# RagnarGrootKoerkamp/astar-pairwise-aligner

Measured on AMD Instinct MI355X. Metric: DP cell-updates/sec (GCUPS), full bit-parallel DP, 100kbp@5% div, higher is better.
Workload: dtype u32

## Files before the change

### astar-pairwise-aligner_amd/csrc/slice_kernel.hpp

```cpp
#pragma once
#include <hip/hip_runtime.h>
#include <stdint.h>

#include "slice_job_order.hpp"

namespace pa {
namespace slice {

#ifndef PA_SLICE_CLOCK_TURNS
#define PA_SLICE_CLOCK_TURNS 15
#endif
#ifndef PA_SLICE_YIELD
#define PA_SLICE_YIELD 2
#endif
constexpr int kPad = 64;
constexpr int kErrSpin = 7;
constexpr uint32_t kSpinLimit = 1u << 22;

struct SliceGroup {
    uint64_t a_off;
    uint64_t b_off;
    uint64_t h_off;
    uint32_t h_stride;
    int32_t n;
    int32_t nstrips;
    int32_t npairs;
    uint32_t first_pos;
    uint32_t ev_first, ev_count;
    uint32_t pad_;
};
struct SliceEvent {
    int32_t col;
    uint32_t mask;
};
struct SlicePair {
    uint64_t a_off, b_off;
    int32_t n, m;
    uint32_t pair;
    uint32_t pad_;
};

typedef uint32_t pa_slice_u32x2 __attribute__((ext_vector_type(2)));
__device__ __forceinline__ uint32_t dpp_wave_shr1(uint32_t old_, uint32_t src) {
    return (uint32_t)__builtin_amdgcn_update_dpp((int)old_, (int)src, 0x138, 0xf, 0xf, false);
}
__device__ __forceinline__ uint32_t dpp_wave_rol1(uint32_t x) {
    return (uint32_t)__builtin_amdgcn_update_dpp((int)x, (int)x, 0x134, 0xf, 0xf, false);
}
__device__ __forceinline__ uint2 ld_boundary(const uint2* p) {
    const unsigned long long v = __hip_atomic_load((const unsigned long long*)p, __ATOMIC_RELAXED, __HIP_MEMORY_SCOPE_AGENT);
    return make_uint2((uint32_t)v, (uint32_t)(v >> 32));
}
__device__ __forceinline__ void st_boundary(uint2* p, uint32_t hp, uint32_t hm) {
    __hip_atomic_store((unsigned long long*)p, (unsigned long long)hp | ((unsigned long long)hm << 32), __ATOMIC_RELAXED, __HIP_MEMORY_SCOPE_AGENT);
}

#define PA_SLICE_ROW_PAIR(vpA, vmA, vpB, vmB, nb0A, nb1A, nb0B, nb1B, a0, a1, hpp, hmp, hpo, hmo)                                      \
    do {                                                                                                                                \
        uint32_t zA_, zB_, hmA_, hpA_;                                                                                                  \
        asm volatile(                                                                                                                   \
            "v_xor_b32 %[zA], %[a1_], %[nb1A_]\n\t"                                                                                     \
            "v_xor_b32 %[zB], %[a1_], %[nb1B_]\n\t"                                                                                     \
            "v_bitop3_b32 %[zA], %[a0_], %[nb0A_], %[zA] bitop3:0x28\n\t"                                                               \
            "v_bitop3_b32 %[zB], %[a0_], %[nb0B_], %[zB] bitop3:0x28\n\t"                                                               \
            "v_bitop3_b32 %[zA], %[zA], %[vmA_], %[hmp_] bitop3:0xfe\n\t"                                                               \
            "v_and_b32 %[hmA], %[zA], %[vpA_]\n\t"                                                                                      \
            "v_bitop3_b32 %[hpA], %[vmA_], %[zA], %[vpA_] bitop3:0xf1\n\t"                                                              \
            "v_bitop3_b32 %[zB], %[zB], %[vmB_], %[hmA] bitop3:0xfe\n\t"                                                                \
            "v_bitop3_b32 %[vpA_], %[hmp_], %[zA], %[hpp_] bitop3:0xf1\n\t"                                                             \
            "v_and_b32 %[hmB], %[zB], %[vpB_]\n\t"                                                                                      \
            "v_and_b32 %[vmA_], %[hpp_], %[zA]\n\t"                                                                                     \
            "v_bitop3_b32 %[hpB], %[vmB_], %[zB], %[vpB_] bitop3:0xf1\n\t"                                                              \
            "v_bitop3_b32 %[vpB_], %[hmA], %[zB], %[hpA] bitop3:0xf1\n\t"                                                               \
            "v_and_b32 %[vmB_], %[hpA], %[zB]"                                                                                          \
            : [zA] "=&v"(zA_), [zB] "=&v"(zB_), [hmA] "=&v"(hmA_), [hpA] "=&v"(hpA_), [hmB] "=&v"(hmo), [hpB] "=&v"(hpo),              \
              [vpA_] "+v"(vpA), [vmA_] "+v"(vmA), [vpB_] "+v"(vpB), [vmB_] "+v"(vmB)                                                    \
            : [a0_] "v"(a0), [a1_] "v"(a1), [nb0A_] "v"(nb0A), [nb1A_] "v"(nb1A), [nb0B_] "v"(nb0B), [nb1B_] "v"(nb1B), [hpp_] "v"(hpp), \
              [hmp_] "v"(hmp));                                                                                                         \
    } while (0)

#define PA_SLICE_ROW_ONE(vpA, vmA, nb0A, nb1A, a0, a1, hpp, hmp, hpo, hmo)                                                              \
    do {                                                                                                                                \
        uint32_t zA_;                                                                                                                   \
        asm volatile(                                                                                                                   \
            "v_xor_b32 %[zA], %[a1_], %[nb1A_]\n\t"                                                                                     \
            "v_bitop3_b32 %[zA], %[a0_], %[nb0A_], %[zA] bitop3:0x28\n\t"                                                               \
            "v_bitop3_b32 %[zA], %[zA], %[vmA_], %[hmp_] bitop3:0xfe\n\t"                                                               \
            "v_and_b32 %[hmA], %[zA], %[vpA_]\n\t"                                                                                      \
            "v_bitop3_b32 %[hpA], %[vmA_], %[zA], %[vpA_] bitop3:0xf1\n\t"                                                              \
            "v_bitop3_b32 %[vpA_], %[hmp_], %[zA], %[hpp_] bitop3:0xf1\n\t"                                                             \
            "v_and_b32 %[vmA_], %[hpp_], %[zA]"                                                                                          \
            : [zA] "=&v"(zA_), [hmA] "=&v"(hmo), [hpA] "=&v"(hpo), [vpA_] "+v"(vpA), [vmA_] "+v"(vmA)                                   \
            : [a0_] "v"(a0), [a1_] "v"(a1), [nb0A_] "v"(nb0A), [nb1A_] "v"(nb1A), [hpp_] "v"(hpp), [hmp_] "v"(hmp));                    \
    } while (0)

constexpr int kRingEntries = 256;
constexpr uint32_t kRingMask = (uint32_t)(kRingEntries - 1) * 16u;

#define PA_SLICE_FEED(hpp, hmp, ohp, ohm, hin, min_)                                                                                     \
    asm volatile(                                                                                                                       \
        "s_mov_b64 vcc, 1\n\t"                                                                                                          \
        "v_cndmask_b32_dpp %[hpp_], %[ohp_], %[hin_], vcc wave_shr:1 row_mask:0xf bank_mask:0xf bound_ctrl:0\n\t"                       \
        "v_cndmask_b32_dpp %[hmp_], %[ohm_], %[hmin_], vcc wave_shr:1 row_mask:0xf bank_mask:0xf bound_ctrl:0"                          \
        : [hpp_] "=&v"(hpp), [hmp_] "=&v"(hmp)                                                                                          \
        : [ohp_] "v"(ohp), [ohm_] "v"(ohm), [hin_] "v"(hin), [hmin_] "v"(min_)                                                          \
        : "vcc")

template <int R>
__global__ __launch_bounds__(64, 2) void slice_kernel(const SliceJob* __restrict__ jobs, int njobs, const SliceGroup* __restrict__ groups,
                                                      const SliceEvent* __restrict__ events, const uint2* __restrict__ A, const uint2* __restrict__ B,
                                                      uint2* H, uint2* V, uint32_t* ticket_err, unsigned long long* dbg) {
    __shared__ uint4 ring[kRingEntries];
    const int lane = (int)threadIdx.x;
    const uint32_t wave_slot = (uint32_t)__builtin_amdgcn_s_getreg((4 - 1) << 11 | 4) & 15u;
    for (;;) {
        uint32_t tk = 0;
        if (lane == 0) tk = atomicAdd(ticket_err, 1u);
        tk = (uint32_t)__builtin_amdgcn_readfirstlane((int)tk);
        if (tk >= (uint32_t)njobs) break;
        const SliceJob job = jobs[tk];
        const SliceGroup grp = groups[job.group];
        const unsigned long long t_job0 = dbg ? __builtin_amdgcn_s_memrealtime() : 0ull;
        unsigned long long t_parked = 0, n_parks = 0;
        [[maybe_unused]] bool waited_before = false;
        [[maybe_unused]] int slack = 0;
        const int s = (int)job.strip, n = grp.n;
        const bool has_in = s > 0, has_out = s + 1 < grp.nstrips;
        const uint2* Ag = A + grp.a_off + kPad;
        const size_t row0 = grp.b_off + ((size_t)s * 64 + (size_t)lane) * R;
        const uint2* Hin = H + grp.h_off + (size_t)(has_in ? s - 1 : 0) * grp.h_stride + kPad;
        uint2* Hout = H + grp.h_off + (size_t)(has_out ? s : 0) * grp.h_stride + kPad;
        const SliceEvent* ev = events + grp.ev_first;
        uint32_t nb0[R], nb1[R], vp[R], vm[R];
#pragma unroll
        for (int i = 0; i < R; ++i) {
            const uint2 b = B[row0 + i];
            nb0[i] = b.x;
            nb1[i] = b.y;
            vp[i] = ~0u;
            vm[i] = 0u;
        }
        constexpr int kWaitStep = 8;
        uint32_t a0 = 0, a1 = 0, o_hp = 0, o_hm = ~0u;
        uint32_t off = (lane == 63 && has_out) ? (uint32_t)(-lane) * 8u : 0x7FFFFFF0u;
        int cnt = 1 - lane;
        int cnt16 = cnt * 16;
        constexpr int kNoEvent = INT32_MIN;
        uint32_t ev_i = 0;
        int ev_col16 = ev[0].col * 16;
        const int nchunks = (n + 63 + 63) / 64;
        const __amdgpu_buffer_rsrc_t hrs = __builtin_amdgcn_make_buffer_rsrc((void*)Hout, 0, (int)((uint32_t)n * 8u), 0x00020000);
        unsigned long long nA = 0, nH = ~0ull;
        uint2 kA = Ag[lane], kH = make_uint2(~0u, 0u);
        if (has_in) kH = ld_boundary(Hin + lane);
        ring[kRingEntries - 64 + lane] = make_uint4(0u, 0u, 0u, ~0u);
        __builtin_amdgcn_s_waitcnt(0);
        for (int q = 0; q < nchunks; ++q) {
#if PA_SLICE_CLOCK_TURNS
            if ((((uint32_t)__builtin_amdgcn_s_memrealtime() >> PA_SLICE_CLOCK_TURNS) ^ wave_slot) & 1u) __builtin_amdgcn_s_setprio(1);
            else __builtin_amdgcn_s_setprio(0);
#else
            if (((uint32_t)q ^ wave_slot) & 1u) __builtin_amdgcn_s_setprio(1);
            else __builtin_amdgcn_s_setprio(0);
#endif
            uint2 cA = kA, cH = kH;
            const int col = q * 64 + lane;
            if (has_in) {
                uint32_t spins = 0;
                const unsigned long long t_p0 = dbg ? __builtin_amdgcn_s_memrealtime() : 0ull;
                while (col < n && (cH.x & cH.y) != 0u) {
                    __builtin_amdgcn_s_sleep(32);
                    cH = ld_boundary(Hin + col);
                    if (++spins > kSpinLimit) {
                        atomicCAS(ticket_err + 1, 0u, (uint32_t)kErrSpin);
                        cH = make_uint2(~0u, 0u);
                    }
                }
                const bool waited = __builtin_amdgcn_readfirstlane((int)(__ballot(spins != 0u) != 0ull)) != 0;
#if PA_SLICE_YIELD == 1
                if (waited) __builtin_amdgcn_s_setprio(0);
#elif PA_SLICE_YIELD == 2
                if (waited || waited_before) __builtin_amdgcn_s_setprio(0);
                waited_before = waited;
#elif PA_SLICE_YIELD >= 3
                slack = waited ? PA_SLICE_YIELD : (slack > 0 ? slack - 1 : 0);
                if (slack > 0) __builtin_amdgcn_s_setprio(0);
#endif
                if (dbg && waited) {
                    t_parked += __builtin_amdgcn_s_memrealtime() - t_p0;
                    n_parks += 1;
                }
                if (col < n) st_boundary(const_cast<uint2*>(Hin) + col, ~0u, ~0u);
            }
            ring[col & (kRingEntries - 1)] = make_uint4(cA.x, cA.y, cH.x, cH.y);
            uint4 r = *(const uint4*)((const char*)ring + ((uint32_t)(cnt16 - 16) & kRingMask));
            const int pcol = min(col + 64, n + kPad - 1);
            const bool more = q + 1 < nchunks;
            if (more) {
                asm volatile("global_load_dwordx2 %0, %1, off ; pa_prefetch_load" : "=v"(nA) : "v"(Ag + pcol) : "memory");
                if (has_in) asm volatile("global_load_dwordx2 %0, %1, off sc1 ; pa_prefetch_load" : "=v"(nH) : "v"(Hin + pcol) : "memory");
            }
            const int jend = min(64, n + 63 - q * 64);
            const int wait_at = more ? kWaitStep : -1;
            for (int j = 0; j < jend; ++j) {
                asm volatile("" : "+s"(j));
                if (j == wait_at) {
                    asm volatile("s_waitcnt vmcnt(8) ; pa_prefetch_wait" : "+v"(nA), "+v"(nH)::"memory");
                    kA = make_uint2((uint32_t)nA, (uint32_t)(nA >> 32));
                    if (has_in) kH = make_uint2((uint32_t)nH, (uint32_t)(nH >> 32));
                }
                uint32_t hpp, hmp;
                a0 = r.x;
                a1 = r.y;
                PA_SLICE_FEED(hpp, hmp, o_hp, o_hm, r.z, r.w);
#pragma unroll
                for (int i = 0; i + 1 < R; i += 2) {
                    uint32_t hpo, hmo;
                    PA_SLICE_ROW_PAIR(vp[i], vm[i], vp[i + 1], vm[i + 1], nb0[i], nb1[i], nb0[i + 1], nb1[i + 1], a0, a1, hpp, hmp, hpo, hmo);
                    hpp = hpo;
                    hmp = hmo;
                }
                if constexpr (R & 1) {
                    uint32_t hpo, hmo;
                    PA_SLICE_ROW_ONE(vp[R - 1], vm[R - 1], nb0[R - 1], nb1[R - 1], a0, a1, hpp, hmp, hpo, hmo);
                    hpp = hpo;
                    hmp = hmo;
                }
                o_hp = hpp;
                o_hm = hmp;
                r = *(const uint4*)((const char*)ring + ((uint32_t)cnt16 & kRingMask));
                {
                    const pa_slice_u32x2 d = {hpp, hmp};
                    __builtin_amdgcn_raw_buffer_store_b64(d, hrs, off, 0, 16);
                }
                off += 8u;
                if (cnt16 == ev_col16) {
                    const uint32_t mask = ev[ev_i].mask;
#pragma unroll
                    for (int i = 0; i < R; ++i) {
                        atomicOr(&V[row0 + i].x, vp[i] & mask);
                        atomicOr(&V[row0 + i].y, vm[i] & mask);
                        asm volatile("" ::: "memory");
                    }
                    ++ev_i;
                    ev_col16 = ev_i < grp.ev_count ? ev[ev_i].col * 16 : kNoEvent;
                    __builtin_amdgcn_s_waitcnt(0);
                }
                cnt16 += 16;
            }
        }
        if (dbg && lane == 0) {
            const unsigned long long dt = __builtin_amdgcn_s_memrealtime() - t_job0;
            atomicMin(dbg + 0, dt);
            atomicMax(dbg + 1, dt);
            atomicAdd(dbg + 2, dt);
            atomicAdd(dbg + 3, 1ull);
            atomicAdd(dbg + 4, t_parked);
            atomicAdd(dbg + 5, n_parks);
            if (s == 0) {
                atomicMin(dbg + 6, dt);
                atomicMax(dbg + 7, dt);
            }
            const uint32_t xcc = (uint32_t)__builtin_amdgcn_s_getreg((4 - 1) << 11 | 20) & 7u;
            atomicAdd(dbg + 8 + 2 * xcc, dt - t_parked);
            atomicAdd(dbg + 9 + 2 * xcc, 1ull);
        }
    }
}


__device__ __forceinline__ uint32_t slice_rank16(const uint4 v, int count, bool& invalid) {
    const uint32_t q[4] = {v.x, v.y, v.z, v.w};
    uint32_t w = 0;
#pragma unroll
    for (int k = 0; k < 16; ++k) {
        const int r = rank_acgt((uint8_t)(q[k >> 2] >> (8 * (k & 3))));
        if (k < count) {
            invalid |= r < 0;
            w |= (uint32_t)(r & 3) << (2 * k);
        }
    }
    return w;
}

__global__ __launch_bounds__(256) void slice_pack_a_kernel(const SliceGroup* __restrict__ groups, const SlicePair* __restrict__ spairs,
                                                           const uint8_t* __restrict__ a_cat, uint2* __restrict__ A, uint32_t* __restrict__ bad) {
    const SliceGroup grp = groups[blockIdx.y];
    const int lane = (int)(threadIdx.x & 63), q = (int)(blockIdx.x * 4 + (threadIdx.x >> 6));
    if ((long long)q * 32 >= (long long)grp.n) return;
    const int p = lane & 31, half = lane >> 5, c0 = 32 * q + 16 * half;
    uint32_t w = 0;
    bool invalid = false;
    if (p < grp.npairs) {
        const SlicePair sp = spairs[grp.first_pos + p];
        if (c0 < sp.n) w = slice_rank16(*(const uint4*)(a_cat + sp.a_off + c0), sp.n - c0, invalid);
    }
    if (invalid) atomicOr(bad, 1u);
    uint32_t a0 = 0, a1 = 0;
#pragma unroll
    for (int k = 0; k < 16; ++k) {
        const unsigned long long b0 = __ballot((w >> (2 * k)) & 1u), b1 = __ballot((w >> (2 * k + 1)) & 1u);
        if ((lane & 15) == k) {
            a0 = (lane & 16) ? (uint32_t)(b0 >> 32) : (uint32_t)b0;
            a1 = (lane & 16) ? (uint32_t)(b1 >> 32) : (uint32_t)b1;
        }
    }
    const int c = q * 32 + lane;
    if (lane < 32 && c < grp.n) A[grp.a_off + kPad + c] = make_uint2(a0, a1);
}

__global__ __launch_bounds__(256) void slice_pack_b_kernel(const SliceGroup* __restrict__ groups, const SlicePair* __restrict__ spairs,
                                                           const uint8_t* __restrict__ b_cat, uint2* __restrict__ B, int rows_per_strip,
                                                           uint32_t* __restrict__ bad) {
    const SliceGroup grp = groups[blockIdx.y];
    const int lane = (int)(threadIdx.x & 63), j = (int)(blockIdx.x * 4 + (threadIdx.x >> 6));
    if ((long long)j * 64 >= (long long)grp.nstrips * rows_per_strip) return;
    const int p = lane & 31, half = lane >> 5;
    const long long r0 = (long long)j * 64 + 32 * half;
    uint32_t x0 = 0, x1 = 0;
    bool invalid = false;
    if (p < grp.npairs) {
        const SlicePair sp = spairs[grp.first_pos + p];
#pragma unroll
        for (int h = 0; h < 2; ++h) {
            const long long r = r0 + 16 * h;
            if (r < (long long)sp.m) {
                const int count = (int)min((long long)sp.m - r, 16ll);
                const uint32_t w = slice_rank16(*(const uint4*)(b_cat + sp.b_off + r), count, invalid);
                const uint32_t real = count >= 16 ? ~0u : (1u << (2 * count)) - 1u, nw = ~w & real;
                uint32_t e = 0, o = 0;
#pragma unroll
                for (int k = 0; k < 16; ++k) {
                    e |= ((nw >> (2 * k)) & 1u) << k;
                    o |= ((nw >> (2 * k + 1)) & 1u) << k;
                }
                x0 |= e << (16 * h);
                x1 |= o << (16 * h);
            }
        }
    }
    if (invalid) atomicOr(bad, 1u);
    uint32_t nb0 = 0, nb1 = 0;
#pragma unroll
    for (int k = 0; k < 32; ++k) {
        const unsigned long long b0 = __ballot((x0 >> k) & 1u), b1 = __ballot((x1 >> k) & 1u);
        if ((lane & 31) == k) {
            nb0 = half ? (uint32_t)(b0 >> 32) : (uint32_t)b0;
            nb1 = half ? (uint32_t)(b1 >> 32) : (uint32_t)b1;
        }
    }
    B[grp.b_off + (size_t)j * 64 + lane] = make_uint2(nb0, nb1);
}

constexpr int kScoreSpan = 4096;
__global__ __launch_bounds__(64) void slice_score_kernel(const SliceGroup* __restrict__ groups, const SlicePair* __restrict__ spairs,
                                                         const uint2* __restrict__ V, int32_t* __restrict__ cost_out) {
    const SliceGroup grp = groups[blockIdx.x];
    const int lane = (int)threadIdx.x;
    int my_m = 0, my_n = 0;
    uint32_t my_pair = 0;
    if (lane < grp.npairs) {
        const SlicePair sp = spairs[grp.first_pos + lane];
        my_m = sp.m;
        my_n = sp.n;
        my_pair = sp.pair;
    }
    int max_m = my_m;
#pragma unroll
    for (int o = 32; o > 0; o >>= 1) max_m = max(max_m, __shfl_xor(max_m, o));
    const int lo = (int)blockIdx.y * kScoreSpan, hi = min(max_m, lo + kScoreSpan);
    if (lo >= max_m) return;
    int acc = blockIdx.y == 0 ? my_n : 0;
    for (int r0 = lo; r0 < hi; r0 += 64) {
        const int r = r0 + lane;
        uint2 v = make_uint2(0u, 0u);
        if (r < hi) v = V[grp.b_off + r];
        for (int p = 0; p < grp.npairs; ++p) {
            const int mp = __shfl(my_m, p);
            const bool in = r < mp;
            const int pos = __popcll(__ballot(in && ((v.x >> p) & 1u))), neg = __popcll(__ballot(in && ((v.y >> p) & 1u)));
            if (lane == p) acc += pos - neg;
        }
    }
    if (lane < grp.npairs && acc != 0) atomicAdd(&cost_out[my_pair], acc);
}

}
}
```

### astar-pairwise-aligner_amd/csrc/slice_unit.hip

```cpp
#include "slice_plan.hpp"

#include <algorithm>
#include <cmath>
#include <cstdio>
#include <cstdlib>
#include <memory>
#include <numeric>
#include <vector>

#include "pa_hip_internal.hpp"
#include "slice_kernel.hpp"

namespace pa {
namespace slice {

struct Plan {
    int R = 52;
    size_t pairs = 0;
    std::vector<SliceGroup> groups;
    std::vector<SliceJob> jobs;
    size_t a_elems = 0, b_elems = 0, h_elems = 0;
    unsigned max_col_blocks = 0, max_row_blocks = 0;
    double valu = 0, computed = 0;
    int chain = 0;
    bool h_dirty = false;
    DeviceBuf d_groups, d_events, d_jobs, d_spairs, d_A, d_B, d_V, d_H;
};

static int strips_for(size_t m, int R) { return (int)((m + (size_t)64 * R - 1) / ((size_t)64 * R)); }

static constexpr double kNsPerRowStep = 16.2, kNsStepOverhead = 11.6, kChainPenalty = 0.0015;

static constexpr int kDefaultChain = 1;
static int chain_setting() {
    const char* e = getenv("PA_SLICE_CHAIN");
    return e && *e ? std::max(0, atoi(e)) : kDefaultChain;
}
static int chain_in_flight(int chain, size_t slots, size_t ngroups, int longest) {
    return chain == 0 ? longest : std::min(std::max(chain, auto_chain(ngroups, longest, slots)), longest);
}

int choose_rows_per_lane(const size_t* a_len, const size_t* b_len, size_t pairs, double simds, double* est_ns) {
    if (const char* e = getenv("PA_SLICE")) {
        if (atoi(e) == 0) return 0;
    }
    size_t live = 0;
    for (size_t i = 0; i < pairs; ++i) {
        live += a_len[i] > 0 && b_len[i] > 0;
        if (a_len[i] >= (size_t(1) << 27) - 64 || b_len[i] >= (size_t(1) << 27)) return 0;
    }
    const bool forced = getenv("PA_SLICE") && atoi(getenv("PA_SLICE")) > 0;
    if ((live + 31) / 32 > 65535) return 0;
    if (live < 64 && !forced) return 0;
    std::vector<uint32_t> order;
    for (size_t i = 0; i < pairs; ++i)
        if (a_len[i] > 0 && b_len[i] > 0) order.push_back((uint32_t)i);
    std::sort(order.begin(), order.end(), [&](uint32_t x, uint32_t y) { return a_len[x] != a_len[y] ? a_len[x] < a_len[y] : (b_len[x] != b_len[y] ? b_len[x] < b_len[y] : x < y); });
    int best_r = 0;
    double best = -1;
    const double slots = simds * 2.0;
    for (const int R : kRowsPerLane) {
        if (forced && atoi(getenv("PA_SLICE")) > 1 && atoi(getenv("PA_SLICE")) != R) continue;
        double work = 0, longest = 0, jobs = 0;
        const size_t ngroups = (order.size() + 31) / 32;
        size_t m_max = 0;
        for (const uint32_t i : order) m_max = std::max(m_max, b_len[i]);
        const int S_max = strips_for(m_max, R);
        const int C = chain_in_flight(chain_setting(), (size_t)slots, ngroups, S_max);
        for (size_t g = 0; g * 32 < order.size(); ++g) {
            size_t n = 0, m = 0;
            for (size_t t = g * 32; t < std::min(order.size(), g * 32 + 32); ++t) {
                n = std::max(n, a_len[order[t]]);
                m = std::max(m, b_len[order[t]]);
            }
            const int S = strips_for(m, R);
            const double per_strip = ((double)n + 63.0) * (R * kNsPerRowStep + kNsStepOverhead) * (1.0 + kChainPenalty * (std::min(S, C) - 1));
            work += per_strip * S;
            jobs += S;
            longest = std::max(longest, per_strip + 128.0 * (S - 1) * (R * kNsPerRowStep + kNsStepOverhead));
        }
        const double waves = std::min(jobs, slots);
        const double speed = waves <= simds ? 1.165 : 1.0 + 0.165 * (slots - waves) / simds;
        const double rounds = jobs > slots ? std::ceil(jobs / slots) * (work / jobs) : work / waves;
        const double t = std::max(longest / 1.165, rounds / speed);
        if (best < 0 || t < best) {
            best = t;
            best_r = R;
        }
    }
    if (est_ns) *est_ns = best;
    return best_r;
}

Plan* create(const size_t* a_len, const size_t* b_len, size_t pairs, const size_t* a_off, const size_t* b_off, int rows_per_lane) {
    auto p = std::make_unique<Plan>();
    p->R = rows_per_lane;
    p->pairs = pairs;
    const int R = rows_per_lane;
    std::vector<uint32_t> order;
    for (size_t i = 0; i < pairs; ++i)
        if (a_len[i] > 0 && b_len[i] > 0) order.push_back((uint32_t)i);
    std::sort(order.begin(), order.end(), [&](uint32_t x, uint32_t y) { return a_len[x] != a_len[y] ? a_len[x] < a_len[y] : (b_len[x] != b_len[y] ? b_len[x] < b_len[y] : x < y); });
    std::vector<SlicePair> spairs(order.size());
    std::vector<SliceEvent> events;
    size_t a_at = 0, b_at = 0, h_at = 0;
    size_t max_n = 0, max_rows = 0;
    const size_t ngroups = (order.size() + 31) / 32;
    for (size_t gi = 0; gi < ngroups; ++gi) {
        const size_t g = ngroups - 1 - gi;
        SliceGroup grp{};
        grp.first_pos = (uint32_t)(g * 32);
        grp.npairs = (int32_t)std::min<size_t>(32, order.size() - g * 32);
        size_t n = 0, m = 0;
        for (int t = 0; t < grp.npairs; ++t) {
            const uint32_t i = order[g * 32 + t];
            n = std::max(n, a_len[i]);
            m = std::max(m, b_len[i]);
            spairs[g * 32 + t] = SlicePair{(uint64_t)a_off[i], (uint64_t)b_off[i], (int32_t)a_len[i], (int32_t)b_len[i], i, 0u};
        }
        grp.n = (int32_t)n;
        grp.nstrips = strips_for(m, R);
        grp.a_off = a_at;
        grp.b_off = b_at;
        grp.h_off = h_at;
        grp.h_stride = (uint32_t)(n + 2 * kPad);
        a_at += n + 2 * kPad;
        b_at += (size_t)grp.nstrips * 64 * R;
        h_at += (size_t)(grp.nstrips - 1) * grp.h_stride;
        grp.ev_first = (uint32_t)events.size();
        for (int t = 0; t < grp.npairs; ++t) {
            const int32_t col = (int32_t)a_len[order[g * 32 + t]];
            if (events.size() > grp.ev_first && events.back().col == col) events.back().mask |= 1u << t;
            else events.push_back(SliceEvent{col, 1u << t});
        }
        grp.ev_count = (uint32_t)events.size() - grp.ev_first;
        max_n = std::max(max_n, n);
        max_rows = std::max(max_rows, (size_t)grp.nstrips * 64 * R);
        p->valu += (double)grp.nstrips * ((double)n + 63.0) * (7.0 * R + kStepOverheadInstr);
        p->computed += (double)grp.nstrips * 64.0 * R * (double)n * 32.0;
        p->groups.push_back(grp);
    }
    {
        std::vector<int> nstrips;
        for (const SliceGroup& g : p->groups) nstrips.push_back(g.nstrips);
        const size_t slots = (size_t)device_cus() * 8;
        p->chain = chain_setting();
        p->jobs = job_order(nstrips, slots, p->chain);
    }
    p->a_elems = a_at;
    p->b_elems = b_at;
    p->h_elems = h_at;
    p->max_col_blocks = (unsigned)((max_n + 127) / 128);
    p->max_row_blocks = (unsigned)((max_rows / 64 + 3) / 4);
    if (p->groups.empty()) return p.release();
    if (events.empty()) events.push_back(SliceEvent{0, 0});
    if (!p->d_groups.alloc(p->groups.size() * sizeof(SliceGroup)) || !p->d_events.alloc(events.size() * sizeof(SliceEvent)) ||
        !p->d_jobs.alloc(p->jobs.size() * sizeof(SliceJob)) || !p->d_spairs.alloc(spairs.size() * sizeof(SlicePair)) || !p->d_A.alloc(a_at * 8) ||
        !p->d_B.alloc(b_at * 8) || !p->d_V.alloc(b_at * 8) || !p->d_H.alloc(std::max<size_t>(h_at, 8) * 8))
        return nullptr;
    if (!hip_ok(hipMemcpy(p->d_groups.ptr, p->groups.data(), p->groups.size() * sizeof(SliceGroup), hipMemcpyHostToDevice), "H2D slice groups") ||
        !hip_ok(hipMemcpy(p->d_events.ptr, events.data(), events.size() * sizeof(SliceEvent), hipMemcpyHostToDevice), "H2D slice events") ||
        !hip_ok(hipMemcpy(p->d_jobs.ptr, p->jobs.data(), p->jobs.size() * sizeof(SliceJob), hipMemcpyHostToDevice), "H2D slice jobs") ||
        !hip_ok(hipMemcpy(p->d_spairs.ptr, spairs.data(), spairs.size() * sizeof(SlicePair), hipMemcpyHostToDevice), "H2D slice pairs") ||
        !hip_ok(hipMemset(p->d_A.ptr, 0, a_at * 8), "memset slice A") ||
        (h_at && !hip_ok(hipMemset(p->d_H.ptr, 0xFF, h_at * 8), "memset slice boundaries")))
        return nullptr;
    return p.release();
}

void destroy(Plan* p) { delete p; }

void mark_clean(Plan* p) { p->h_dirty = false; }

template <int R>
static hipError_t launch_slice(int grid, hipStream_t s, const Plan* p, uint32_t* d_ticket_err, unsigned long long* dbg) {
    hipLaunchKernelGGL((slice_kernel<R>), dim3((unsigned)grid), dim3(64), 0, s, p->d_jobs.as<SliceJob>(), (int)p->jobs.size(), p->d_groups.as<SliceGroup>(),
                       p->d_events.as<SliceEvent>(), p->d_A.as<uint2>(), p->d_B.as<uint2>(), p->d_H.as<uint2>(), p->d_V.as<uint2>(), d_ticket_err, dbg);
    return hipGetLastError();
}

int run(Plan* p, hipStream_t s, const uint8_t* d_a, const uint8_t* d_b, uint32_t* d_bad, int32_t* d_costs, uint32_t* d_ticket_err, hipEvent_t ev0,
        hipEvent_t ev1) {
    if (!hip_ok(hipMemsetAsync(d_ticket_err, 0, 8, s), "memset slice ticket")) return PA_E_HIP;
    if (p->groups.empty()) {
        if (ev0 && (!hip_ok(hipEventRecord(ev0, s), "event") || !hip_ok(hipEventRecord(ev1, s), "event"))) return PA_E_HIP;
        return 0;
    }
    const unsigned G = (unsigned)p->groups.size();
    hipLaunchKernelGGL(slice_pack_a_kernel, dim3(p->max_col_blocks, G), dim3(256), 0, s, p->d_groups.as<SliceGroup>(), p->d_spairs.as<SlicePair>(), d_a,
                       p->d_A.as<uint2>(), d_bad);
    hipLaunchKernelGGL(slice_pack_b_kernel, dim3(p->max_row_blocks, G), dim3(256), 0, s, p->d_groups.as<SliceGroup>(), p->d_spairs.as<SlicePair>(), d_b,
                       p->d_B.as<uint2>(), 64 * p->R, d_bad);
    if (!hip_ok(hipGetLastError(), "slice transposes")) return PA_E_HIP;
    if (!hip_ok(hipMemsetAsync(p->d_V.ptr, 0, p->b_elems * 8, s), "memset slice V")) return PA_E_HIP;
    if (p->h_elems && p->h_dirty && !hip_ok(hipMemsetAsync(p->d_H.ptr, 0xFF, p->h_elems * 8, s), "memset slice boundaries")) return PA_E_HIP;
    p->h_dirty = true;
    int grid = (int)std::min<size_t>(p->jobs.size(), (size_t)device_cus() * 8);
    const int grid_cap = getenv("PA_SLICE_GRID") ? atoi(getenv("PA_SLICE_GRID")) : 0;
    if (grid_cap > 0) grid = std::min(grid, grid_cap);
    static const bool jobtimes = getenv("PA_SLICE_JOBTIMES") != nullptr;
    unsigned long long* dbg = nullptr;
    if (jobtimes && hipMalloc((void**)&dbg, 192) == hipSuccess) {
        const unsigned long long init[24] = {~0ull, 0, 0, 0, 0, 0, ~0ull, 0};
        if (hipMemcpyAsync(dbg, init, 192, hipMemcpyHostToDevice, s) != hipSuccess || hipStreamSynchronize(s) != hipSuccess) dbg = nullptr;
    }
    if (ev0 && !hip_ok(hipEventRecord(ev0, s), "event")) return PA_E_HIP;
    hipError_t e = hipSuccess;
    switch (p->R) {
        case 52: e = launch_slice<52>(grid, s, p, d_ticket_err, dbg); break;
        case 51: e = launch_slice<51>(grid, s, p, d_ticket_err, dbg); break;
        case 50: e = launch_slice<50>(grid, s, p, d_ticket_err, dbg); break;
        case 49: e = launch_slice<49>(grid, s, p, d_ticket_err, dbg); break;
        case 48: e = launch_slice<48>(grid, s, p, d_ticket_err, dbg); break;
        case 47: e = launch_slice<47>(grid, s, p, d_ticket_err, dbg); break;
        case 46: e = launch_slice<46>(grid, s, p, d_ticket_err, dbg); break;
        case 45: e = launch_slice<45>(grid, s, p, d_ticket_err, dbg); break;
        case 44: e = launch_slice<44>(grid, s, p, d_ticket_err, dbg); break;
        case 42: e = launch_slice<42>(grid, s, p, d_ticket_err, dbg); break;
        case 40: e = launch_slice<40>(grid, s, p, d_ticket_err, dbg); break;
        case 36: e = launch_slice<36>(grid, s, p, d_ticket_err, dbg); break;
        case 32: e = launch_slice<32>(grid, s, p, d_ticket_err, dbg); break;
        case 28: e = launch_slice<28>(grid, s, p, d_ticket_err, dbg); break;
        default: set_error("slice: no kernel for %d rows per lane", p->R); return PA_E_INTERNAL;
    }
    if (!hip_ok(e, "slice_kernel")) return PA_E_HIP;
    if (ev1 && !hip_ok(hipEventRecord(ev1, s), "event")) return PA_E_HIP;
    if (dbg) {
        unsigned long long h[24] = {0};
        if (hipMemcpyAsync(h, dbg, 192, hipMemcpyDeviceToHost, s) == hipSuccess && hipStreamSynchronize(s) == hipSuccess && h[3]) {
            std::fprintf(stderr, "[slice jobs] awake us per job by XCD:");
            for (int x = 0; x < 8; ++x) std::fprintf(stderr, " %d: %.0f (%llu)", x, h[9 + 2 * x] ? h[8 + 2 * x] * 0.01 / (double)h[9 + 2 * x] : 0.0, h[9 + 2 * x]);
            std::fprintf(stderr, "\n");
            std::fprintf(stderr, "[slice jobs] R %d chain %d: %llu jobs, us per job: min %.1f mean %.1f max %.1f (first strips: min %.1f max %.1f); asleep behind the strip above: %.2f %% of the job time, %.1f waits per job\n",
                         p->R, p->chain, h[3], h[0] * 0.01, h[2] * 0.01 / (double)h[3], h[1] * 0.01, h[6] * 0.01, h[7] * 0.01, 100.0 * (double)h[4] / (double)h[2], (double)h[5] / (double)h[3]);
        }
        (void)hipFree(dbg);
    }
    hipLaunchKernelGGL(slice_score_kernel, dim3(G, (p->max_row_blocks * 256u + kScoreSpan - 1) / kScoreSpan), dim3(64), 0, s, p->d_groups.as<SliceGroup>(), p->d_spairs.as<SlicePair>(), p->d_V.as<uint2>(), d_costs);
    if (!hip_ok(hipGetLastError(), "slice_score_kernel")) return PA_E_HIP;
    return 0;
}

Info info(const Plan* p) {
    Info i{};
    i.rows_per_lane = p->R;
    i.groups = p->groups.size();
    i.jobs = p->jobs.size();
    i.chain = p->chain;
    i.valu_instructions = p->valu;
    i.computed_rows_cells = p->computed;
    i.device_bytes = (double)(p->a_elems + 2 * p->b_elems + p->h_elems) * 8.0;
    i.boundary_bytes = (double)p->h_elems * 8.0;
    return i;
}

}
}
```

Before: 274,100.

## Use SWAR base ranking and swizzle-based 32x32 bit transpose in pack and score kernels

```diff
diff --git a/astar-pairwise-aligner_amd/csrc/slice_kernel.hpp b/astar-pairwise-aligner_amd/csrc/slice_kernel.hpp
--- a/astar-pairwise-aligner_amd/csrc/slice_kernel.hpp
+++ b/astar-pairwise-aligner_amd/csrc/slice_kernel.hpp
@@ -268,99 +268,130 @@
     }
 }
 
-
-__device__ __forceinline__ uint32_t slice_rank16(const uint4 v, int count, bool& invalid) {
-    const uint32_t q[4] = {v.x, v.y, v.z, v.w};
-    uint32_t w = 0;
-#pragma unroll
-    for (int k = 0; k < 16; ++k) {
-        const int r = rank_acgt((uint8_t)(q[k >> 2] >> (8 * (k & 3))));
-        if (k < count) {
-            invalid |= r < 0;
-            w |= (uint32_t)(r & 3) << (2 * k);
-        }
-    }
-    return w;
+#define PA_SLICE_T32_STAGES(X) X(16, 0x0000FFFFu) X(8, 0x00FF00FFu) X(4, 0x0F0F0F0Fu) X(2, 0x33333333u) X(1, 0x55555555u)
+
+template <int D>
+__device__ __forceinline__ uint32_t slice_t32_stage(uint32_t x, uint32_t keep_clear, int lane) {
+    const uint32_t y = (uint32_t)__builtin_amdgcn_ds_swizzle((int)x, (D << 10) | 0x1f);
+    const bool set = (lane & D) != 0;
+    const uint32_t keep = set ? ~keep_clear : keep_clear;
+    const uint32_t moved = __builtin_amdgcn_alignbit(y, y, set ? (uint32_t)D : (uint32_t)(32 - D));
+    return (x & keep) | (moved & ~keep);
+}
+__device__ __forceinline__ uint32_t slice_transpose32(uint32_t x, int lane) {
+#define PA_SLICE_T32_STAGE_(D, KEEP) x = slice_t32_stage<D>(x, KEEP, lane);
+    PA_SLICE_T32_STAGES(PA_SLICE_T32_STAGE_)
+#undef PA_SLICE_T32_STAGE_
+    return x;
+}
+
+constexpr int kPackTile = 128;
+
+__device__ __forceinline__ uint32_t slice_rank4(uint32_t x) {
+    const uint32_t s1 = x >> 1, s2 = x >> 2;
+    const uint32_t t = s2 & ~s1 & 0x01010101u;
+    const uint32_t letter = ((((x & 0x06060606u) | 0x41414141u) ^ t) | (t << 4));
+    const uint32_t d = x ^ letter;
+    const uint32_t bad = ((((d & 0x7f7f7f7fu) + 0x7f7f7f7fu) | d) >> 7) & 0x01010101u;
+    const uint32_t c0 = ((s1 ^ s2) & 0x01010101u) | bad, c1 = (s2 & 0x01010101u) | bad;
+    return (((c0 | (c1 << 4)) * 0x01020408u) >> 24) | (((bad * 0x01020408u) >> 24) << 8);
+}
+
+struct SliceTileBits {
+    uint32_t c0[2], c1[2], bad[2], valid[2];
+};
+__device__ __forceinline__ SliceTileBits slice_read_tile(const uint8_t* __restrict__ seq, int len, int pos0) {
+    uint4 v[4];
+#pragma unroll
+    for (int i = 0; i < 4; ++i) {
+        const int pos = pos0 + 64 * (i >> 1) + 16 * (i & 1);
+        v[i] = make_uint4(0u, 0u, 0u, 0u);
+        if (pos < len) v[i] = *(const uint4*)(seq + pos);
+    }
+    SliceTileBits t;
+#pragma unroll
+    for (int j = 0; j < 2; ++j) {
+        uint32_t c0 = 0, c1 = 0, bad = 0;
+#pragma unroll
+        for (int h = 0; h < 2; ++h) {
+            const uint32_t q[4] = {v[2 * j + h].x, v[2 * j + h].y, v[2 * j + h].z, v[2 * j + h].w};
+#pragma unroll
+            for (int k = 0; k < 4; ++k) {
+                const uint32_t r = slice_rank4(q[k]);
+                c0 |= (r & 15u) << (16 * h + 4 * k);
+                c1 |= ((r >> 4) & 15u) << (16 * h + 4 * k);
+                bad |= (r >> 8) << (16 * h + 4 * k);
+            }
+        }
+        const int left = min(max(len - (pos0 + 64 * j), 0), 32);
+        t.c0[j] = c0;
+        t.c1[j] = c1;
+        t.bad[j] = bad;
+        t.valid[j] = left >= 32 ? ~0u : (1u << left) - 1u;
+    }
+    return t;
 }
 
 __global__ __launch_bounds__(256) void slice_pack_a_kernel(const SliceGroup* __restrict__ groups, const SlicePair* __restrict__ spairs,
                                                            const uint8_t* __restrict__ a_cat, uint2* __restrict__ A, uint32_t* __restrict__ bad) {
     const SliceGroup grp = groups[blockIdx.y];
-    const int lane = (int)(threadIdx.x & 63), q = (int)(blockIdx.x * 4 + (threadIdx.x >> 6));
-    if ((long long)q * 32 >= (long long)grp.n) return;
-    const int p = lane & 31, half = lane >> 5, c0 = 32 * q + 16 * half;
-    uint32_t w = 0;
-    bool invalid = false;
+    const int lane = (int)(threadIdx.x & 63);
+    const long long tile = (long long)blockIdx.x * 4 + (threadIdx.x >> 6);
+    if (tile * kPackTile >= (long long)grp.n) return;
+    const int c_tile = (int)tile * kPackTile, p = lane & 31, half = lane >> 5;
+    int len = 0;
+    const uint8_t* seq = a_cat;
     if (p < grp.npairs) {
         const SlicePair sp = spairs[grp.first_pos + p];
-        if (c0 < sp.n) w = slice_rank16(*(const uint4*)(a_cat + sp.a_off + c0), sp.n - c0, invalid);
-    }
-    if (invalid) atomicOr(bad, 1u);
-    uint32_t a0 = 0, a1 = 0;
-#pragma unroll
-    for (int k = 0; k < 16; ++k) {
-        const unsigned long long b0 = __ballot((w >> (2 * k)) & 1u), b1 = __ballot((w >> (2 * k + 1)) & 1u);
-        if ((lane & 15) == k) {
-            a0 = (lane & 16) ? (uint32_t)(b0 >> 32) : (uint32_t)b0;
-            a1 = (lane & 16) ? (uint32_t)(b1 >> 32) : (uint32_t)b1;
-        }
-    }
-    const int c = q * 32 + lane;
-    if (lane < 32 && c < grp.n) A[grp.a_off + kPad + c] = make_uint2(a0, a1);
+        len = sp.n;
+        seq = a_cat + sp.a_off;
+    }
+    const SliceTileBits t = slice_read_tile(seq, len, c_tile + 32 * half);
+    if (((t.bad[0] & t.valid[0]) | (t.bad[1] & t.valid[1])) != 0u) atomicOr(bad, 1u);
+#pragma unroll
+    for (int j = 0; j < 2; ++j) {
+        const uint32_t a0 = slice_transpose32(t.c0[j] & t.valid[j], lane), a1 = slice_transpose32(t.c1[j] & t.valid[j], lane);
+        const int c = c_tile + 64 * j + lane;
+        if (c < grp.n) A[grp.a_off + kPad + c] = make_uint2(a0, a1);
+    }
 }
 
 __global__ __launch_bounds__(256) void slice_pack_b_kernel(const SliceGroup* __restrict__ groups, const SlicePair* __restrict__ spairs,
                                                            const uint8_t* __restrict__ b_cat, uint2* __restrict__ B, int rows_per_strip,
                                                            uint32_t* __restrict__ bad) {
     const SliceGroup grp = groups[blockIdx.y];
-    const int lane = (int)(threadIdx.x & 63), j = (int)(blockIdx.x * 4 + (threadIdx.x >> 6));
-    if ((long long)j * 64 >= (long long)grp.nstrips * rows_per_strip) return;
-    const int p = lane & 31, half = lane >> 5;
-    const long long r0 = (long long)j * 64 + 32 * half;
-    uint32_t x0 = 0, x1 = 0;
-    bool invalid = false;
+    const int lane = (int)(threadIdx.x & 63);
+    const long long tile = (long long)blockIdx.x * 4 + (threadIdx.x >> 6);
+    const long long rows = (long long)grp.nstrips * rows_per_strip;
+    if (tile * kPackTile >= rows) return;
+    const int r_tile = (int)tile * kPackTile, p = lane & 31, half = lane >> 5;
+    int len = 0;
+    const uint8_t* seq = b_cat;
     if (p < grp.npairs) {
         const SlicePair sp = spairs[grp.first_pos + p];
-#pragma unroll
-        for (int h = 0; h < 2; ++h) {
-            const long long r = r0 + 16 * h;
-            if (r < (long long)sp.m) {
-                const int count = (int)min((long long)sp.m - r, 16ll);
-                const uint32_t w = slice_rank16(*(const uint4*)(b_cat + sp.b_off + r), count, invalid);
-                const uint32_t real = count >= 16 ? ~0u : (1u << (2 * count)) - 1u, nw = ~w & real;
-                uint32_t e = 0, o = 0;
-#pragma unroll
-                for (int k = 0; k < 16; ++k) {
-                    e |= ((nw >> (2 * k)) & 1u) << k;
-                    o |= ((nw >> (2 * k + 1)) & 1u) << k;
-                }
-                x0 |= e << (16 * h);
-                x1 |= o << (16 * h);
-            }
-        }
-    }
-    if (invalid) atomicOr(bad, 1u);
-    uint32_t nb0 = 0, nb1 = 0;
-#pragma unroll
-    for (int k = 0; k < 32; ++k) {
-        const unsigned long long b0 = __ballot((x0 >> k) & 1u), b1 = __ballot((x1 >> k) & 1u);
-        if ((lane & 31) == k) {
-            nb0 = half ? (uint32_t)(b0 >> 32) : (uint32_t)b0;
-            nb1 = half ? (uint32_t)(b1 >> 32) : (uint32_t)b1;
-        }
-    }
-    B[grp.b_off + (size_t)j * 64 + lane] = make_uint2(nb0, nb1);
+        len = sp.m;
+        seq = b_cat + sp.b_off;
+    }
+    const SliceTileBits t = slice_read_tile(seq, len, r_tile + 32 * half);
+    if (((t.bad[0] & t.valid[0]) | (t.bad[1] & t.valid[1])) != 0u) atomicOr(bad, 1u);
+#pragma unroll
+    for (int j = 0; j < 2; ++j) {
+        const uint32_t nb0 = slice_transpose32(~t.c0[j] & t.valid[j], lane), nb1 = slice_transpose32(~t.c1[j] & t.valid[j], lane);
+        const long long r = (long long)r_tile + 64 * j + lane;
+        if (r < rows) B[grp.b_off + (size_t)r] = make_uint2(nb0, nb1);
+    }
 }
 
 constexpr int kScoreSpan = 4096;
+constexpr int kScoreReads = 4;
 __global__ __launch_bounds__(64) void slice_score_kernel(const SliceGroup* __restrict__ groups, const SlicePair* __restrict__ spairs,
                                                          const uint2* __restrict__ V, int32_t* __restrict__ cost_out) {
     const SliceGroup grp = groups[blockIdx.x];
-    const int lane = (int)threadIdx.x;
+    const int lane = (int)threadIdx.x, p = lane & 31, half = lane >> 5;
     int my_m = 0, my_n = 0;
     uint32_t my_pair = 0;
-    if (lane < grp.npairs) {
-        const SlicePair sp = spairs[grp.first_pos + lane];
+    if (p < grp.npairs) {
+        const SlicePair sp = spairs[grp.first_pos + p];
         my_m = sp.m;
         my_n = sp.n;
         my_pair = sp.pair;
@@ -370,18 +401,24 @@
     for (int o = 32; o > 0; o >>= 1) max_m = max(max_m, __shfl_xor(max_m, o));
     const int lo = (int)blockIdx.y * kScoreSpan, hi = min(max_m, lo + kScoreSpan);
     if (lo >= max_m) return;
-    int acc = blockIdx.y == 0 ? my_n : 0;
-    for (int r0 = lo; r0 < hi; r0 += 64) {
-        const int r = r0 + lane;
-        uint2 v = make_uint2(0u, 0u);
-        if (r < hi) v = V[grp.b_off + r];
-        for (int p = 0; p < grp.npairs; ++p) {
-            const int mp = __shfl(my_m, p);
-            const bool in = r < mp;
-            const int pos = __popcll(__ballot(in && ((v.x >> p) & 1u))), neg = __popcll(__ballot(in && ((v.y >> p) & 1u)));
-            if (lane == p) acc += pos - neg;
-        }
-    }
+    int acc = (blockIdx.y == 0 && half == 0) ? my_n : 0;
+    for (int r0 = lo; r0 < hi; r0 += 64 * kScoreReads) {
+        uint2 v[kScoreReads];
+#pragma unroll
+        for (int u = 0; u < kScoreReads; ++u) {
+            const int r = r0 + 64 * u + lane;
+            v[u] = make_uint2(0u, 0u);
+            if (r < hi) v[u] = V[grp.b_off + r];
+        }
+#pragma unroll
+        for (int u = 0; u < kScoreReads; ++u) {
+            const uint32_t tp = slice_transpose32(v[u].x, lane), tm = slice_transpose32(v[u].y, lane);
+            const int left = min(max(my_m - (r0 + 64 * u + 32 * half), 0), 32);
+            const uint32_t valid = left >= 32 ? ~0u : (1u << left) - 1u;
+            acc += __popc(tp & valid) - __popc(tm & valid);
+        }
+    }
+    acc += __shfl_xor(acc, 32);
     if (lane < grp.npairs && acc != 0) atomicAdd(&cost_out[my_pair], acc);
 }
 
diff --git a/astar-pairwise-aligner_amd/csrc/slice_unit.hip b/astar-pairwise-aligner_amd/csrc/slice_unit.hip
--- a/astar-pairwise-aligner_amd/csrc/slice_unit.hip
+++ b/astar-pairwise-aligner_amd/csrc/slice_unit.hip
@@ -21,6 +21,7 @@
     std::vector<SliceJob> jobs;
     size_t a_elems = 0, b_elems = 0, h_elems = 0;
     unsigned max_col_blocks = 0, max_row_blocks = 0;
+    size_t max_rows = 0;
     double valu = 0, computed = 0;
     int chain = 0;
     bool h_dirty = false;
@@ -150,8 +151,9 @@
     p->a_elems = a_at;
     p->b_elems = b_at;
     p->h_elems = h_at;
-    p->max_col_blocks = (unsigned)((max_n + 127) / 128);
-    p->max_row_blocks = (unsigned)((max_rows / 64 + 3) / 4);
+    p->max_col_blocks = (unsigned)((max_n + 4 * kPackTile - 1) / (4 * kPackTile));
+    p->max_row_blocks = (unsigned)((max_rows + 4 * kPackTile - 1) / (4 * kPackTile));
+    p->max_rows = max_rows;
     if (p->groups.empty()) return p.release();
     if (events.empty()) events.push_back(SliceEvent{0, 0});
     if (!p->d_groups.alloc(p->groups.size() * sizeof(SliceGroup)) || !p->d_events.alloc(events.size() * sizeof(SliceEvent)) ||
@@ -236,7 +238,7 @@
         }
         (void)hipFree(dbg);
     }
-    hipLaunchKernelGGL(slice_score_kernel, dim3(G, (p->max_row_blocks * 256u + kScoreSpan - 1) / kScoreSpan), dim3(64), 0, s, p->d_groups.as<SliceGroup>(), p->d_spairs.as<SlicePair>(), p->d_V.as<uint2>(), d_costs);
+    hipLaunchKernelGGL(slice_score_kernel, dim3(G, (unsigned)((p->max_rows + kScoreSpan - 1) / kScoreSpan)), dim3(64), 0, s, p->d_groups.as<SliceGroup>(), p->d_spairs.as<SlicePair>(), p->d_V.as<uint2>(), d_costs);
     if (!hip_ok(hipGetLastError(), "slice_score_kernel")) return PA_E_HIP;
     return 0;
 }
```

After: 276,500 (median of 6 runs). No clear change (+0.9%).
